# YuxiaWu/RAG4DyG

Measured on AMD Instinct MI355X. Metric: query-seqs/sec encode+top-k over full pool, higher is better.
Workload: dtype f32 (f16x2 operands: two fp16 terms, three products, f32 accumulate)

## Files before the change

rag4dyg_amd/csrc/common.h:

```cpp
#pragma once
#include <hip/hip_runtime.h>
#include <stdint.h>
#include <stdio.h>
#include <stdarg.h>
#include "../../include/r4d.h"
#include "conv1d_route.h"

namespace r4d {

void set_error(const char* fmt, ...);
int dbgflag_kc(); int dbgflag_att(); int dbgflag_sk(); int dbgflag_jac(); int dbgflag_scan(); int dbgflag_s3(); int dbgflag_h2();

#define R4D_REQUIRE(cond, ...)                     \
    do {                                           \
        if (!(cond)) {                             \
            r4d::set_error(__VA_ARGS__);           \
            return R4D_ERR_INVALID;                \
        }                                          \
    } while (0)

#define R4D_HIP(call)                                                                  \
    do {                                                                               \
        hipError_t e_ = (call);                                                        \
        if (e_ != hipSuccess) {                                                        \
// ... 100 lines not shown
bool gemm_skinny_fuses_ln(int M, int K, int N);
void* gemm_skinny_counters(float* scratch, size_t* bytes);
int launch_gemm_skinny(const float* x, const float* wT, const float* bias, const float* resid, int M, int K, int N,
                       int epilogue, float* y, float* scratch, hipStream_t s, const float* ln_w = nullptr,
                       const float* ln_b = nullptr, float ln_eps = 0.f, bool counters_zeroed = false, const float* ln_fold = nullptr);
int launch_fold_layernorm(const float* wT, const float* g, const float* beta, int N, int K, float* wTg, float* lnc, hipStream_t s);

struct S3Args {
    const float* A; const unsigned short* planes; float* C;
    const float* bias; const float* resid;
    int M, N, K, lda, ldc, ldr, epilogue;
    unsigned* kblk; int kb_hd;
};
static inline S3Args s3_args(const float* x, const unsigned short* planes, const float* bias, const float* resid, int M, int K, int N,
                             int epilogue, float* y) {
    S3Args a{};
    a.A = x; a.planes = planes; a.C = y; a.bias = bias; a.resid = resid;
    a.M = M; a.N = N; a.K = K; a.lda = K; a.ldc = N; a.ldr = N; a.epilogue = epilogue;
    return a;
}
int launch_gemm_s3(const S3Args& a, hipStream_t stream);
bool gemm_s3_f32b_supported(int M, int K, int N);
int launch_gemm_s3_f32b(const float* A, const float* B, float* C, int M, int N, int K, int lda, int ldc, int epilogue, hipStream_t stream);
int launch_gemm_s3_scan_order(const float* q_hat, const float* pool_hat, float* scores, int Q, int N, int d, int ng, hipStream_t stream);
int launch_gemm_h2(const S3Args& a, hipStream_t stream);
int launch_split2_planes(const float* w, int N, int K, long long ld_k, long long ld_n, unsigned short* planes, hipStream_t s);
extern int g_gemm_h2p;
bool gemm_h2p_supported(int M, int K, int N);
int launch_gemm_h2p(const S3Args& a, const unsigned short* a_lines, bool out_lines, hipStream_t stream);
int launch_split2_lines(const float* x, long long rows, int K, unsigned short* lines, hipStream_t s);
int launch_gemm_b1(const S3Args& a, hipStream_t stream);
int launch_gemm_b1tn(const float* X, const float* dY, float* out, float* db_out, int I, int J, int M, int lda, int ldb, int S,
                     hipStream_t stream);
int launch_gemm_b1h(const GemmArgs& g, hipStream_t stream);
int launch_gemm_s3tn(const float* X, const float* dY, float* out, float* db_partials, int I, int J, int M, int lda, int ldb, int S,
                     hipStream_t stream);
static inline int gemm_tn_slices(int I, int J, int M, int max_slices) {
    const int tiles = (I / 128) * (J / 256);
    int S = cdiv(512, tiles);
    const int smax = cdiv(M, 256);
    if (S > smax) S = smax;
    if (S > max_slices) S = max_slices;
    return S < 1 ? 1 : S;
}
static inline int tn_row_slices(int M, int S) { return cdiv(M, cdiv(cdiv(M, S), 32) * 32); }
int launch_splitk_reduce(const float* part, long long n4, int S, float* C, hipStream_t stream);
extern int g_encode_bf16;
// ... 39 lines not shown
struct LMLayout { size_t train, h, logits, dh, dwte, tn, ce, total; };
LMLayout lm_layout(const r4d_gpt2_config* cfg, int B, int T, int ldV);
int head_train_step(const char* who, const r4d_gpt2_config* cfg, const r4d_gpt2_weights* w, const r4d_gpt2_grads* grads,
                    const r4d_lm_head* head, int head_mode, float* head_grad, const int64_t* ids_d, const SpliceIn* sp, int B, int T,
                    float gscale, float* loss, float* d_fused, float* hidden_out, const r4d_train_dropout* dropout, void* workspace_d,
                    size_t workspace_bytes, hipStream_t s);

template <typename T> size_t topk_ws_bytes(int rows, int n, int k);
template <typename T>
int topk_rows(const T* vals, const long long* idx_in, int rows, int n, long long ld, int k, long long index_offset, T* out_v,
              long long* out_i, void* ws, size_t ws_bytes, bool counters_zeroed, hipStream_t s);

int launch_layernorm(const float* x, const float* w, const float* b, int rows, int d, float eps, float* y,
                     hipStream_t s);
bool layernorm_lines_supported(int d);
int launch_layernorm_lines(const float* x, const float* w, const float* b, int rows, int d, float eps, unsigned short* y_lines, hipStream_t s);
constexpr int ATT_MAXG = 16;
struct RowGroups {
    int n;
    int B[ATT_MAXG], T[ATT_MAXG];
    const int64_t* ids[ATT_MAXG];
    const float* emb[ATT_MAXG];
};
int launch_embed_layernorm_groups(const RowGroups& G, const float* wte, const float* wpe, int vocab, int d,
                                  const float* w, const float* b, float eps, float* x_out, float* y_out, hipStream_t s, bool y_lines = false);
int launch_causal_softmax(float* S, int nbh, int T, int ld, int row_tile, hipStream_t s);
int launch_embed_pos_layernorm(const int64_t* ids, const float* emb, const int32_t* pos, const float* wte,
                               const float* wpe, int vocab, int n_positions, int t_cap, int B, int d, const float* w,
                               const float* b, float eps, float* x_out, float* y_out, hipStream_t s,
                               void* zero_words = nullptr, size_t zero_bytes = 0);
int launch_decode_attention(const float* qkv_new, float* kv_layer, const int32_t* pos, int B, int t_cap, int H, int d,
                            float* out, hipStream_t s);
struct GreedyState {
    int64_t* next; int32_t* lens; int32_t* pos; int32_t* active; int32_t* gen_len; int32_t* out_tokens;
    const int32_t* params;
    int out_cap, t_cap;
};
struct GreedyEmbed { const float* wte; const float* wpe; float* x_out; unsigned* zero_words; int vocab, n_positions, d, n_zero; };
int launch_greedy_advance(const float* logits, int B, int V, const GreedyState& st, hipStream_t s, const GreedyEmbed* embed = nullptr);
struct AttnGroups {
    int n;
    int seq_prefix[ATT_MAXG + 1];
    int T[ATT_MAXG];
    long long row0[ATT_MAXG];
};
bool attention_h2_supported(int H, int d);
int launch_attention_h2_groups(const unsigned* qkv_words, int n, const int* Bs, const int* Ts, const long long* row0s, int H, int d,
                               float* out, hipStream_t s, bool out_lines = false, const unsigned* kblk = nullptr);
// ... 7 lines not shown
extern int g_attention_variant;
extern int g_attention_fused;
constexpr int PAD_ROWS_HDR = 8;
struct PadRowsPlan {
    int M, Mp, Tmax, Tcap, nblk, ntab, lmax, vocab;
    size_t words() const { return (size_t)PAD_ROWS_HDR + 2 * (size_t)Tcap + lmax + nblk + 2 * (size_t)Mp + vocab; }
    size_t rows() const { return (size_t)Mp + Tcap; }
};
static inline PadRowsPlan pad_rows_plan(size_t M, int Tmax, int vocab) {
    PadRowsPlan p;
    p.M = (int)M; p.Mp = (int)((M + 31) / 32 * 32); p.Tmax = Tmax; p.Tcap = (Tmax + 31) / 32 * 32;
    p.nblk = p.Mp / 32; p.ntab = p.Tcap / 32; p.lmax = (p.nblk + p.ntab + 3) / 4 * 4; p.vocab = vocab;
    return p;
}
struct PadRowsBuf {
    int* hdr; long long* tab_ids; int *list, *drop, *tok, *pos, *hist;
};
static inline PadRowsBuf pad_rows_buf(int* hdr, const PadRowsPlan& p) {
    PadRowsBuf b;
    b.hdr = hdr; b.tab_ids = reinterpret_cast<long long*>(hdr + PAD_ROWS_HDR);
    b.tok = hdr + PAD_ROWS_HDR + 2 * p.Tcap; b.pos = b.tok + p.Mp; b.list = b.pos + p.Mp; b.drop = b.list + p.lmax; b.hist = b.drop + p.nblk;
    return b;
}
int launch_pad_rows_gather(const RowGroups& G, int vocab, long long row_base, const PadRowsBuf& b, hipStream_t s);
int launch_pad_rows_classify(const PadRowsPlan& p, const PadRowsBuf& b, hipStream_t s);
int launch_pad_rows_fill(const PadRowsPlan& p, const PadRowsBuf& b, unsigned* qkv_words, unsigned* kblk, int d, hipStream_t s);
int launch_gemm_h2p_rowmap(const S3Args& a, const unsigned short* a_lines, const PadRowsPlan& p, const PadRowsBuf& b, hipStream_t stream);
constexpr int LNF_ROWS_PER_CHUNK = 16;
size_t lnf_meanpool_scratch_floats(int B, int T, int d);
int launch_lnf_meanpool_groups(const RowGroups& G, const float* x, const float* w, const float* b, int d, float eps,
                               float* hidden_out, float* pool_out, float* scratch, hipStream_t s);

}
```

rag4dyg_amd/csrc/encoder.hip:

```cpp
#include <math.h>
#include <stdlib.h>
#include <string.h>
#include <vector>
#include "common.h"

namespace r4d {

static thread_local char g_err[512] = "";
void set_error(const char* fmt, ...) {
    va_list ap;
    va_start(ap, fmt);
    vsnprintf(g_err, sizeof(g_err), fmt, ap);
    va_end(ap);
}

int g_gemm_split3 = 1;
int g_encode_bf16 = 0;

int conv1d(const Conv1DW& W, const float* x, const float* resid, int M, int epilogue, float* y, hipStream_t s, const Conv1DOpts& opts) {
    const int K = W.in, N = W.out;
    const GemmRoute route = conv1d_route(W, M, epilogue, opts.skinny_scratch != nullptr, opts.bf16);
    switch (route) {
        case ROUTE_B1:
            if (opts.bf16 == BF16_TRAIN) R4D_BRANCH(TB_FWD);
// ... 250 lines not shown
        const r4d_gpt2_layer& L = w->layers[l];
        R4D_REQUIRE(L.ln_1_w && L.c_attn_w && L.attn_proj_w && L.ln_2_w && L.c_fc_w && L.mlp_proj_w,
                    "gpt2: null weight in layer %d", l);
        const Conv1DW Wqkv = conv1d_w(L, C_ATTN, d), Wo = conv1d_w(L, ATTN_PROJ, d), Wfc = conv1d_w(L, C_FC, d), Wp = conv1d_w(L, MLP_PROJ, d);
        const Conv1DOpts enc{nullptr, false, g_encode_bf16 ? BF16_ENCODE : BF16_OFF};
        const bool lines = !g_encode_bf16 && g_gemm_split3 == 2 && g_gemm_h2p && Wqkv.h2 && Wfc.h2 && Wp.h2 && layernorm_lines_supported(d) &&
                           gemm_h2p_supported(M, d, 3 * d) && gemm_h2p_supported(M, d, 4 * d) && gemm_h2p_supported(M, 4 * d, d);
        unsigned short* ln_lines = reinterpret_cast<unsigned short*>(ws.ln);
        unsigned short* fc_lines = reinterpret_cast<unsigned short*>(ws.fc);
        float* qkv = out_qkv_d ? out_qkv_d + (size_t)l * M * 3 * d : ws.qkv;
        bool words = !g_encode_bf16 && !out_qkv_d && g_attention_h2 && g_attention_fused != 0 && g_gemm_split3 == 2 && Wqkv.h2 &&
                     attention_h2_supported(H, d) && gemm_h2_supported(M, d, 3 * d);
        int Bs[ATT_MAXG], Ts[ATT_MAXG], nseq;
        long long r0[ATT_MAXG];
        for (int g0 = 0; g0 < n_groups && words; g0 += ATT_MAXG) {
            attn_chunk(groups, g0, n_groups, Bs, Ts, r0, &nseq);
            if (nseq > 65535) words = false;
        }
        if (g_attention_kblk < 0) { const char* e = getenv("R4D_ATT_KBLK"); g_attention_kblk = e ? atoi(e) != 0 : 1; }
        const bool kblk = words && lines && g_attention_kblk && (d / H) % 32 == 0;
        const bool pad0 = l == 0 && kblk && all_ids && layer0_pad_rows_on() && (3 * d) % 256 == 0 && gemm_h2p_supported((int)pr.rows(), d, 3 * d) &&
                          pr.rows() <= 0x7fffffff / (size_t)(16 * d);
        const PadRowsBuf pb = pad_rows_buf(ws.pad_rows, pr);
        if (pad0) {
            if (hipMemsetAsync(pb.hist, 0, (size_t)pr.vocab * sizeof(int), s) != hipSuccess) { set_error("gpt2: memset of the token counts failed"); return R4D_ERR_HIP; }
            for (int g0 = 0; g0 < n_groups; g0 += ATT_MAXG)
                if ((rc = launch_pad_rows_gather(row_groups(groups, g0, n_groups), cfg->vocab, (long long)groups[g0].row0, pb, s))) return rc;
            if ((rc = launch_pad_rows_classify(pr, pb, s))) return rc;
        }
        if (l == 0) {
            for (int g0 = 0; g0 < n_groups; g0 += ATT_MAXG) {
                const RowGroups R = row_groups(groups, g0, n_groups);
                const size_t r0 = groups[g0].row0;
                rc = launch_embed_layernorm_groups(R, w->wte, w->wpe, cfg->vocab, d, L.ln_1_w, L.ln_1_b, cfg->ln_eps,
                                                   ws.x + r0 * d, ws.ln + r0 * d, s, lines);
                if (rc) return rc;
            }
            if (pad0) {
                RowGroups R = {};
                R.n = 1; R.B[0] = 1; R.T[0] = pr.Tmax; R.ids[0] = reinterpret_cast<const int64_t*>(pb.tab_ids);
                if ((rc = launch_embed_layernorm_groups(R, w->wte, w->wpe, cfg->vocab, d, L.ln_1_w, L.ln_1_b, cfg->ln_eps,
                                                        ws.x + (size_t)pr.Mp * d, ws.ln + (size_t)pr.Mp * d, s, lines))) return rc;
            }
        } else if ((rc = lines ? launch_layernorm_lines(ws.x, L.ln_1_w, L.ln_1_b, M, d, cfg->ln_eps, ln_lines, s)
                               : launch_layernorm(ws.x, L.ln_1_w, L.ln_1_b, M, d, cfg->ln_eps, ws.ln, s))) {
            return rc;
        }
        if (out_layers_d &&
            hipMemcpyAsync(out_layers_d + (size_t)l * M * d, ws.x, (size_t)M * d * sizeof(float),
                           hipMemcpyDeviceToDevice, s) != hipSuccess) {
            set_error("gpt2: layer copy failed");
            return R4D_ERR_HIP;
        }
// ... 338 lines not shown
```

rag4dyg_amd/csrc/encoder_ops.hip:

```cpp
#include <string.h>
#include "common.h"
#include "h2.h"

namespace r4d {

constexpr int MAXV = 32;

__device__ __forceinline__ float wave_sum(float v) {
#pragma unroll
    for (int o = 32; o > 0; o >>= 1) v += __shfl_xor(v, o, 64);
    return v;
}
__device__ __forceinline__ float wave_max(float v) {
#pragma unroll
    for (int o = 32; o > 0; o >>= 1) v = fmaxf(v, __shfl_xor(v, o, 64));
    return v;
}

__device__ __forceinline__ void ln_row(float (&v)[MAXV], int nv, int d, float eps) {
    float s = 0.f;
#pragma unroll
    for (int i = 0; i < MAXV; ++i) if (i < nv) s += v[i];
    const float mean = wave_sum(s) / (float)d;
    float q = 0.f;
// ... 133 lines not shown
    const float* src;
    bool bad = false;
    if (in.ids[g]) {
        const long long id = in.ids[g][local];
        bad = id < 0 || id >= vocab;
        src = wte + (bad ? 0 : id) * (long long)d;
    } else {
        src = in.emb[g] + local * d;
    }
    const float* pe = wpe + (local % G.T[g]) * d;
#pragma unroll
    for (int i = 0; i < MAXV; ++i)
        if (i < nv) {
            const float e = src[lane + 64 * i] + pe[lane + 64 * i];
            v[i] = bad ? __builtin_nanf("") : e;
            x_out[row * d + lane + 64 * i] = v[i];
        }
    ln_row(v, nv, d, eps);
#pragma unroll
    for (int i = 0; i < MAXV; ++i)
        if (i < nv) y_out[row * d + lane + 64 * i] = v[i] * w[lane + 64 * i] + b[lane + 64 * i];
}

template <int NQ, bool LINES = false>
__global__ __launch_bounds__(256) void embed_ln4_groups_kernel(const RowTable G, const RowInputs in,
                                                               const float* __restrict__ wte, const float* __restrict__ wpe,
                                                               int vocab, int d, const float* __restrict__ w,
                                                               const float* __restrict__ b, float eps,
                                                               float* __restrict__ x_out, float* __restrict__ y_out) {
    const int lane = threadIdx.x & 63;
    const long long row = (long long)blockIdx.x * 4 + (threadIdx.x >> 6);
    if (row >= G.row_prefix[G.n]) return;
    int g = 0;
    while (g + 1 < G.n && row >= G.row_prefix[g + 1]) ++g;
    const long long local = row - G.row_prefix[g];
    const int nq = d >> 8;
    const float* src;
    bool bad = false;
    if (in.ids[g]) {
        const long long id = in.ids[g][local];
        bad = id < 0 || id >= vocab;
        src = wte + (bad ? 0 : id) * (long long)d;
    } else {
        src = in.emb[g] + local * d;
    }
    const float4* s4 = reinterpret_cast<const float4*>(src) + lane;
    const float4* p4 = reinterpret_cast<const float4*>(wpe + (local % G.T[g]) * d) + lane;
    float4* xr = reinterpret_cast<float4*>(x_out + row * d) + lane;
    float4 v[NQ];
#pragma unroll
    for (int i = 0; i < NQ; ++i) {
        v[i] = make_float4(0.f, 0.f, 0.f, 0.f);
        if (i < nq) {
            const float4 e = s4[64 * i], q = p4[64 * i];
            const float nan = __builtin_nanf("");
            v[i] = bad ? make_float4(nan, nan, nan, nan) : make_float4(e.x + q.x, e.y + q.y, e.z + q.z, e.w + q.w);
            xr[64 * i] = v[i];
        }
    }
    float s_ = 0.f;
#pragma unroll
    for (int i = 0; i < NQ; ++i) s_ += (v[i].x + v[i].y) + (v[i].z + v[i].w);
    const float mean = wave_sum(s_) / (float)d;
    float q = 0.f;
#pragma unroll
    for (int i = 0; i < NQ; ++i)
        if (i < nq) {
            const float a0 = v[i].x - mean, a1 = v[i].y - mean, a2 = v[i].z - mean, a3 = v[i].w - mean;
            q += (a0 * a0 + a1 * a1) + (a2 * a2 + a3 * a3);
        }
    const float rstd = rsqrtf(wave_sum(q) / (float)d + eps);
    float4* yr = reinterpret_cast<float4*>(y_out + row * d) + lane;
#pragma unroll
    for (int i = 0; i < NQ; ++i)
        if (i < nq) {
            const float4 ww = reinterpret_cast<const float4*>(w)[lane + 64 * i], bb = reinterpret_cast<const float4*>(b)[lane + 64 * i];
            const float4 y4 = make_float4((v[i].x - mean) * rstd * ww.x + bb.x, (v[i].y - mean) * rstd * ww.y + bb.y,
                                          (v[i].z - mean) * rstd * ww.z + bb.z, (v[i].w - mean) * rstd * ww.w + bb.w);
            if constexpr (LINES) store_lines4(y_out, row, d, 4 * lane + 256 * i, y4.x, y4.y, y4.z, y4.w);
            else yr[64 * i] = y4;
        }
}

int launch_embed_layernorm_groups(const RowGroups& G, const float* wte, const float* wpe, int vocab, int d,
                                  const float* w, const float* b, float eps, float* x_out, float* y_out, hipStream_t s, bool y_lines) {
    R4D_REQUIRE(d % 64 == 0 && d <= 64 * MAXV, "embed: d=%d must be a multiple of 64 and <= %d", d, 64 * MAXV);
    R4D_REQUIRE(G.n >= 1 && G.n <= ATT_MAXG, "embed: %d batches per launch (max %d)", G.n, ATT_MAXG);
    const RowTable t = make_table(G);
    const long long rows = t.row_prefix[G.n];
    if (rows <= 0) return R4D_OK;
    RowInputs in;
    for (int g = 0; g < ATT_MAXG; ++g) { in.ids[g] = g < G.n ? G.ids[g] : nullptr; in.emb[g] = g < G.n ? G.emb[g] : nullptr; }
    ProfScope prof(PK_EMBED_LN, 12.0 * rows * d + 8.0 * rows, s);
    uintptr_t align = (uintptr_t)wte | (uintptr_t)wpe | (uintptr_t)w | (uintptr_t)b | (uintptr_t)x_out | (uintptr_t)y_out;
    for (int g = 0; g < G.n; ++g) align |= (uintptr_t)in.emb[g];
    const bool vec = d % 256 == 0 && (align & 15) == 0;
    const dim3 grid((unsigned)cdiv(rows, 4));
    if (y_lines) {
        R4D_REQUIRE(vec, "embed: line output needs d %% 256 == 0 and 16-byte aligned pointers");
        R4D_BRANCH(EMBED_LN4);
        if (d <= 512) hipLaunchKernelGGL((embed_ln4_groups_kernel<2, true>), grid, dim3(256), 0, s, t, in, wte, wpe, vocab, d, w, b, eps, x_out, y_out);
        else if (d <= 1024) hipLaunchKernelGGL((embed_ln4_groups_kernel<4, true>), grid, dim3(256), 0, s, t, in, wte, wpe, vocab, d, w, b, eps, x_out, y_out);
        else hipLaunchKernelGGL((embed_ln4_groups_kernel<8, true>), grid, dim3(256), 0, s, t, in, wte, wpe, vocab, d, w, b, eps, x_out, y_out);
        R4D_CHECK_LAUNCH("embed_layernorm");
        return R4D_OK;
    }
    if (vec && d <= 512) { R4D_BRANCH(EMBED_LN4); hipLaunchKernelGGL(embed_ln4_groups_kernel<2>, grid, dim3(256), 0, s, t, in, wte, wpe, vocab, d, w, b, eps, x_out, y_out); }
    else if (vec && d <= 1024) { R4D_BRANCH(EMBED_LN4); hipLaunchKernelGGL(embed_ln4_groups_kernel<4>, grid, dim3(256), 0, s, t, in, wte, wpe, vocab, d, w, b, eps, x_out, y_out); }
    else if (vec) { R4D_BRANCH(EMBED_LN4); hipLaunchKernelGGL(embed_ln4_groups_kernel<8>, grid, dim3(256), 0, s, t, in, wte, wpe, vocab, d, w, b, eps, x_out, y_out); }
    else {
        R4D_BRANCH(EMBED_GENERIC);
        hipLaunchKernelGGL(embed_ln_groups_kernel, grid, dim3(256), 0, s, t, in, wte, wpe, vocab, d, w, b, eps, x_out, y_out);
    }
    R4D_CHECK_LAUNCH("embed_layernorm");
    return R4D_OK;
}

__global__ __launch_bounds__(256) void embed_pos_ln_kernel(const int64_t* __restrict__ ids, const float* __restrict__ emb,
                                                           const int32_t* __restrict__ pos, const float* __restrict__ wte,
                                                           const float* __restrict__ wpe, int vocab, int n_positions,
                                                           int t_cap, int B, int d, const float* __restrict__ w,
                                                           const float* __restrict__ b, float eps,
                                                           float* __restrict__ x_out, float* __restrict__ y_out,
                                                           unsigned* __restrict__ zero_words, int n_zero) {
    if (blockIdx.x == 0)
        for (int i = threadIdx.x; i < n_zero; i += 256) zero_words[i] = 0u;
    const int lane = threadIdx.x & 63;
    const int row = blockIdx.x * 4 + (threadIdx.x >> 6);
    if (row >= B) return;
    const int nv = d >> 6;
    const int p = pos[row];
    bool bad = p < 0 || p >= n_positions || p >= t_cap;
// ... 354 lines not shown
        else hipLaunchKernelGGL(lnf_partial_kernel<32>, grid, dim3(256), 4 * d * sizeof(float), s, t, x, w, b, d, eps, hidden_out, part, g_range_flag);
        R4D_CHECK_LAUNCH("lnf_partial");
    }
    if (pool_out) {
        ProfScope prof(PK_MEANPOOL_REDUCE, 4.0 * parts * d + 4.0 * nseq * d, s);
        hipLaunchKernelGGL(meanpool_reduce_kernel, dim3(nseq), dim3(256), 0, s, t, scratch, d, pool_out);
        R4D_CHECK_LAUNCH("meanpool_reduce");
    }
    return R4D_OK;
}

__global__ __launch_bounds__(256) void pad_rows_gather_kernel(const RowTable G, const RowInputs in, int vocab, long long row_base,
                                                              int* __restrict__ tok, int* __restrict__ pos, int* __restrict__ hist) {
    const long long row = (long long)blockIdx.x * 256 + threadIdx.x;
    if (row >= G.row_prefix[G.n]) return;
    int g = 0;
    while (g + 1 < G.n && row >= G.row_prefix[g + 1]) ++g;
    const long long local = row - G.row_prefix[g];
    const long long id = in.ids[g][local];
    const bool ok = id >= 0 && id < vocab;
    const int t = (int)(local % G.T[g]);
    tok[row_base + row] = ok ? (int)id : -1;
    pos[row_base + row] = t;
    if (ok && t == G.T[g] - 1) atomicAdd(&hist[id], 1);
}

__global__ __launch_bounds__(1024) void pad_rows_classify_kernel(const PadRowsPlan p, const PadRowsBuf b) {
    __shared__ unsigned long long red[1024];
    __shared__ int scan[1024];
    __shared__ int base[2];
    const int tid = threadIdx.x;
    unsigned long long best = 0;
    for (int v = tid; v < p.vocab; v += 1024) {
        const unsigned long long key = ((unsigned long long)(unsigned)b.hist[v] << 32) | (0xffffffffu - (unsigned)v);
        best = key > best ? key : best;
    }
    red[tid] = best;
    if (tid == 0) { base[0] = 0; base[1] = 0; }
    __syncthreads();
    for (int o = 512; o > 0; o >>= 1) {
        if (tid < o) red[tid] = red[tid + o] > red[tid] ? red[tid + o] : red[tid];
        __syncthreads();
    }
    const int c = (int)(0xffffffffu - (unsigned)(red[0] & 0xffffffffu));
    for (int t = tid; t < p.Tcap; t += 1024) b.tab_ids[t] = c;
    for (int b0 = 0; b0 < p.nblk; b0 += 1024) {
        const int blk = b0 + tid;
        bool kept = false, in = blk < p.nblk;
        if (in) {
            kept = blk * 32 + 32 > p.M;
            if (!kept) {
                const int4* t4 = reinterpret_cast<const int4*>(b.tok + blk * 32);
#pragma unroll
                for (int i = 0; i < 8; ++i) { const int4 v = t4[i]; kept |= (v.x != c) | (v.y != c) | (v.z != c) | (v.w != c); }
            }
        }
        scan[tid] = kept ? 1 : 0;
// ... 23 lines not shown
    }
}

__global__ __launch_bounds__(256) void pad_rows_fill_kernel(const PadRowsPlan p, const PadRowsBuf b, uint4* __restrict__ qkv,
                                                            uint4* __restrict__ kblk, int d) {
    if ((int)blockIdx.x >= b.hdr[1]) return;
    const int blk = b.drop[blockIdx.x];
    __shared__ int prow[32];
    if (threadIdx.x < 32) prow[threadIdx.x] = p.Mp + min(b.pos[blk * 32 + threadIdx.x], p.Tcap - 1);
    __syncthreads();
    const int dq = d / 4;
    for (int i = threadIdx.x; i < 32 * dq; i += 256) {
        const int r = i / dq, j = i - r * dq;
        const long long dst = (long long)(blk * 32 + r) * (3 * dq) + j, src = (long long)prow[r] * (3 * dq) + j;
        qkv[dst] = qkv[src];
        qkv[dst + 2 * dq] = qkv[src + 2 * dq];
    }
    for (int i = threadIdx.x; i < 32 * dq; i += 256) {
        const int ch = i >> 5, r = i & 31, sr = prow[r];
        kblk[((long long)blk * dq + ch) * 32 + r] = kblk[((long long)(sr >> 5) * dq + ch) * 32 + (sr & 31)];
    }
}

int launch_pad_rows_gather(const RowGroups& G, int vocab, long long row_base, const PadRowsBuf& b, hipStream_t s) {
    R4D_REQUIRE(G.n >= 1 && G.n <= ATT_MAXG, "pad_rows: %d batches per launch (max %d)", G.n, ATT_MAXG);
    const RowTable t = make_table(G);
    const long long rows = t.row_prefix[G.n];
    if (rows <= 0) return R4D_OK;
    RowInputs in;
    for (int g = 0; g < ATT_MAXG; ++g) { in.ids[g] = g < G.n ? G.ids[g] : nullptr; in.emb[g] = nullptr; }
    for (int g = 0; g < G.n; ++g) R4D_REQUIRE(in.ids[g], "pad_rows: batches given as embeddings have no tokens to classify");
    ProfScope prof(PK_PAD_CLASSIFY, 16.0 * rows, s);
    hipLaunchKernelGGL(pad_rows_gather_kernel, dim3((unsigned)cdiv(rows, 256)), dim3(256), 0, s, t, in, vocab, row_base, b.tok, b.pos, b.hist);
    R4D_CHECK_LAUNCH("pad_rows_gather");
    return R4D_OK;
}

int launch_pad_rows_classify(const PadRowsPlan& p, const PadRowsBuf& b, hipStream_t s) {
    ProfScope prof(PK_PAD_CLASSIFY, 4.0 * p.Mp + 4.0 * p.vocab + 8.0 * p.nblk, s);
    hipLaunchKernelGGL(pad_rows_classify_kernel, dim3(1), dim3(1024), 0, s, p, b);
    R4D_CHECK_LAUNCH("pad_rows_classify");
    return R4D_OK;
}

int launch_pad_rows_fill(const PadRowsPlan& p, const PadRowsBuf& b, unsigned* qkv_words, unsigned* kblk, int d, hipStream_t s) {
    R4D_REQUIRE(qkv_words && kblk && d % 32 == 0 && ((((uintptr_t)qkv_words | (uintptr_t)kblk)) & 15) == 0, "pad_rows_fill: bad arguments");
    ProfScope prof(PK_PAD_FILL, 24.0 * p.Mp * d, s);
    hipLaunchKernelGGL(pad_rows_fill_kernel, dim3(p.nblk), dim3(256), 0, s, p, b, reinterpret_cast<uint4*>(qkv_words),
                       reinterpret_cast<uint4*>(kblk), d);
    R4D_CHECK_LAUNCH("pad_rows_fill");
    return R4D_OK;
}

}
```

rag4dyg_amd/csrc/gemm_s3.hip:

```cpp
#include <stdlib.h>
#include <string.h>
#include <atomic>
#include "bf16x3.h"

#ifndef S3_NRS
#define S3_NRS 1
#endif
#ifndef S3_DBG
#define S3_DBG 0
#endif

namespace r4d {

struct S3Shape {
    int M, N, K, lda, ldc, ldr;
    int plane_bytes;
};

__global__ __launch_bounds__(256) void split3_planes_kernel(const float* __restrict__ w, int N, int K, long long ld_k,
                                                            long long ld_n, unsigned short* __restrict__ planes) {
    __shared__ float tile[32][33];
    const int n0 = blockIdx.x * 32, k0 = blockIdx.y * 32;
    const int tx = threadIdx.x & 31, ty = threadIdx.x >> 5;
    const bool n_fast = ld_n == 1;
// ... 18 lines not shown

template <int BM, int BN, int WGM, int WGN, int NBUF, int NRS, int EPI, bool BF32 = false, int SCAN = 0>
__global__ __launch_bounds__(64 * WGM * WGN, (WGM * WGN) / 4) void gemm_s3_kernel(
    const float* __restrict__ Ag, const unsigned short* __restrict__ Bp, float* __restrict__ Cg,
    const float* __restrict__ biasg, const float* __restrict__ residg, const S3Shape g) {
    constexpr int BK = 32;
    constexpr int NTHREADS = 64 * WGM * WGN;
    constexpr int WM = BM / WGM, WN = BN / WGN, TM = WM / 32, TN = WN / 32;
    constexpr int NIA = BM * 4 / NTHREADS, NIB = BN * 4 / NTHREADS;
    constexpr int A_PLANE = BM * 4, B_PLANE = BN * 4;
    constexpr int STAGE = 3 * (A_PLANE + B_PLANE);
    constexpr int D = NBUF - 1;
    static_assert(NIA >= 1 && NIB >= 1 && NIA <= 2 && NIB <= 2 && TM >= 1 && TN >= 1 && (NBUF == 2 || NBUF == 3), "tile");
    static_assert(NRS == 1 || (NRS == 2 && NBUF == 2), "two register stages: with the two-stage LDS ring only");
    __shared__ u32x4 lds[NBUF * STAGE];

    int m0, n0;
    grouped_tile<BM, BN>(g.M, g.N, m0, n0);
    const int nkt = g.K / BK;

    const int tid = threadIdx.x, lane = tid & 63, wid = tid >> 6;
    const int wm = wid / WGN, wn = wid % WGN;
    const int li = lane & 31, lh = lane >> 5;

    int a_off[NIA], b_off[NIB], a_dst[NIA], b_dst[NIB];
#pragma unroll
    for (int i = 0; i < NIA; ++i) {
        const int idx = tid + i * NTHREADS, row = idx >> 2, c = idx & 3;
        a_off[i] = (min(m0 + row, g.M - 1) * g.lda + (SCAN ? (c >> 1) * 16 + (c & 1) * 4 : c * 8)) * 4;
        a_dst[i] = row * 4 + (c ^ ((row >> 2) & 3));
    }
#pragma unroll
    for (int i = 0; i < NIB; ++i) {
        const int idx = tid + i * NTHREADS, row = idx >> 2, c = idx & 3;
        b_off[i] = (min(n0 + row, g.N - 1) * g.K + (SCAN ? (c >> 1) * 16 + (c & 1) * 4 : c * 8)) * (BF32 ? 4 : 2);
        b_dst[i] = row * 4 + (c ^ ((row >> 2) & 3));
    }
    const __amdgpu_buffer_rsrc_t a_rsrc = __builtin_amdgcn_make_buffer_rsrc(
        const_cast<float*>(Ag), 0, (int)(((long long)(g.M - 1) * g.lda + g.K) * 4), 0x00020000);
    const __amdgpu_buffer_rsrc_t b_rsrc = __builtin_amdgcn_make_buffer_rsrc(
        const_cast<unsigned short*>(Bp), 0, BF32 ? (int)((long long)g.N * g.K * 4) : 3 * g.plane_bytes, 0x00020000);

    u32x4 ra[NRS][NIA][2], rb[NRS][NIB][3];
    static_assert(SCAN == 0 || BF32, "scan order: with the fp32 second operand only");
    constexpr int P2 = SCAN ? 32 : 16;
    const int scan_kw = SCAN ? nkt / (SCAN ? SCAN : 1) : 1;
// ... 420 lines not shown
}

bool gemm_s3_f32b_supported(int M, int K, int N) {
    return gemm_s3_supported(M, K, N) && (long long)N * K * 4 < (1ll << 31);
}
int launch_gemm_s3_f32b(const float* A, const float* B, float* C, int M, int N, int K, int lda, int ldc, int epilogue, hipStream_t stream) {
    R4D_REQUIRE(A && B && C && gemm_s3_f32b_supported(M, K, N), "gemm_s3_f32b: unsupported shape M=%d K=%d N=%d", M, K, N);
    R4D_REQUIRE(lda % 4 == 0 && ((uintptr_t)A % 16) == 0 && ((uintptr_t)B % 16) == 0, "gemm_s3_f32b: alignment");
    R4D_BRANCH(S3_F32B);
    const int tiles = cdiv(M, 128) * cdiv(N, 256);
    ProfScope prof(PK_GEMM_S3_128x256, 2.0 * (double)M * N * K, stream);
    S3Shape sh;
    sh.M = M; sh.N = N; sh.K = K; sh.lda = lda; sh.ldc = ldc; sh.ldr = ldc; sh.plane_bytes = 0;
    const unsigned short* Bp = reinterpret_cast<const unsigned short*>(B);
    if (epilogue == EPI_HALF_PLUS)
        hipLaunchKernelGGL((gemm_s3_kernel<128, 256, 2, 4, 2, 1, EPI_HALF_PLUS, true>), dim3(tiles), dim3(512), 0, stream, A, Bp, C, nullptr, nullptr, sh);
    else if (epilogue == EPI_NONE)
        hipLaunchKernelGGL((gemm_s3_kernel<128, 256, 2, 4, 2, 1, EPI_NONE, true>), dim3(tiles), dim3(512), 0, stream, A, Bp, C, nullptr, nullptr, sh);
    else { set_error("gemm_s3_f32b: epilogue %d has no instantiation", epilogue); return R4D_ERR_INVALID; }
    R4D_CHECK_LAUNCH("gemm_s3_f32b");
    return R4D_OK;
}

int launch_gemm_s3_scan_order(const float* q_hat, const float* pool_hat, float* scores, int Q, int N, int d, int ng, hipStream_t stream) {
    if (!gemm_s3_f32b_supported(Q, d, N) || ng < 2 || ng > 4 || (d / 32) % ng != 0) return 1;
    if ((((uintptr_t)q_hat | (uintptr_t)pool_hat) & 15u) != 0 || d % 4 != 0) return 1;
    R4D_BRANCH(SCAN_TILED);
    const int tiles = cdiv(Q, 128) * cdiv(N, 256);
    S3Shape sh;
    sh.M = Q; sh.N = N; sh.K = d; sh.lda = d; sh.ldc = N; sh.ldr = N; sh.plane_bytes = 0;
    const unsigned short* Bp = reinterpret_cast<const unsigned short*>(pool_hat);
#define S3_SCAN_LAUNCH_(NG_) hipLaunchKernelGGL((gemm_s3_kernel<128, 256, 2, 4, 2, 1, EPI_HALF_PLUS, true, NG_>), dim3(tiles), dim3(512), 0, stream, q_hat, Bp, scores, nullptr, nullptr, sh)
    switch (ng) {
        case 2: S3_SCAN_LAUNCH_(2); break;
        case 3: S3_SCAN_LAUNCH_(3); break;
        default: S3_SCAN_LAUNCH_(4); break;
    }
#undef S3_SCAN_LAUNCH_
    R4D_CHECK_LAUNCH("gemm_s3_scan_order");
    return R4D_OK;
}

int launch_split3_planes(const float* w, int N, int K, long long ld_k, long long ld_n, unsigned short* planes, hipStream_t s) {
    R4D_REQUIRE(w && planes && N >= 1 && K >= 1, "split3_planes: bad arguments");
    R4D_REQUIRE(ld_n == 1 || ld_k == 1, "split3_planes: one of the two strides must be 1");
    hipLaunchKernelGGL(split3_planes_kernel, dim3(cdiv(N, 32), cdiv(K, 32)), dim3(256), 0, s, w, N, K, ld_k, ld_n, planes);
    R4D_CHECK_LAUNCH("split3_planes");
    return R4D_OK;
}

int dbgflag_s3() { return S3_DBG != 0; }

}

using namespace r4d;
// ... 15 lines not shown
```

rag4dyg_amd/csrc/score.hip:

```cpp
#include <math.h>
#include <string.h>
#include <stdlib.h>
#include "bf16x3.h"

#ifndef SCAN_RING_P
#define SCAN_RING_P 3
#endif
#ifndef SCAN_DBG
#define SCAN_DBG 0
#endif

namespace r4d {

int dbgflag_scan() { return SCAN_DBG != 0; }

__global__ __launch_bounds__(256) void normalize_rows_kernel(const float* __restrict__ x, int n, int d,
                                                             float* __restrict__ out, unsigned* __restrict__ range_flag) {
    const int lane = threadIdx.x & 63;
    const int row = blockIdx.x * 4 + (threadIdx.x >> 6);
    if (row >= n) return;
    const float* p = x + (long long)row * d;
    float s = 0.f;
    for (int c = lane; c < d; c += 64) s += p[c] * p[c];
#pragma unroll
// ... 683 lines not shown
    }
    R4D_CHECK_LAUNCH("pool_scan");
    return R4D_OK;
}

template <int KW, int NG>
static int launch_scan_variant(const float* qhat, const float* pool, int Q, int N, float* scores, unsigned* zero_d, int nzero,
                               hipStream_t s) {
    if (g_gemm_split3) { R4D_BRANCH(SCAN_BF16X3); return launch_scan_variant_p<KW, NG, true>(qhat, pool, Q, N, scores, zero_d, nzero, s); }
    R4D_BRANCH(SCAN_F32);
    return launch_scan_variant_p<KW, NG, false>(qhat, pool, Q, N, scores, zero_d, nzero, s);
}

static int launch_pool_scan(const float* qhat, const float* pool, int Q, int N, int d, float* scores, unsigned* zero_d,
                            int nzero, hipStream_t s) {
    static int kw8 = -1;
    if (kw8 < 0) { const char* e = getenv("R4D_SCAN_KW8"); kw8 = e ? atoi(e) : 1; }
    if (d != 32 && d != 64 && d != 128 && d != 256 && d != 384 && d != 512 && d != 768 && d != 1024) return 1;
    ProfScope prof(PK_POOL_SCAN, 4.0 * N * d * cdiv(Q, 32) + 4.0 * Q * d + 4.0 * (double)Q * N, s);
    static int tiled = -1;
    if (tiled < 0) { const char* e = getenv("R4D_SCAN_TILED"); tiled = e ? atoi(e) : 1; }
    if (tiled && Q >= 64 && g_gemm_split3 && (long long)cdiv(Q, 128) * cdiv(N, 256) >= 192) {
        const int ng = d == 256 ? 2 : d == 384 ? 3 : d == 512 ? (kw8 ? 2 : 4) : d == 768 ? 3 : d == 1024 ? 4 : 1;
        if (nzero > 0) R4D_HIP(hipMemsetAsync(zero_d, 0, (size_t)nzero * sizeof(unsigned), s));
        const int rc = launch_gemm_s3_scan_order(qhat, pool, scores, Q, N, d, ng, s);
        if (rc <= 0) return rc;
    }
    switch (d) {
        case 32:   R4D_BRANCH(SCAN_1_1); return launch_scan_variant<1, 1>(qhat, pool, Q, N, scores, zero_d, nzero, s);
        case 64:   R4D_BRANCH(SCAN_2_1); return launch_scan_variant<2, 1>(qhat, pool, Q, N, scores, zero_d, nzero, s);
        case 128:  R4D_BRANCH(SCAN_4_1); return launch_scan_variant<4, 1>(qhat, pool, Q, N, scores, zero_d, nzero, s);
        case 256:  R4D_BRANCH(SCAN_4_2); return launch_scan_variant<4, 2>(qhat, pool, Q, N, scores, zero_d, nzero, s);
        case 384:  R4D_BRANCH(SCAN_4_3); return launch_scan_variant<4, 3>(qhat, pool, Q, N, scores, zero_d, nzero, s);
        case 512:  if (kw8) { R4D_BRANCH(SCAN_8_2); return launch_scan_variant<8, 2>(qhat, pool, Q, N, scores, zero_d, nzero, s); }
                   R4D_BRANCH(SCAN_4_4); return launch_scan_variant<4, 4>(qhat, pool, Q, N, scores, zero_d, nzero, s);
        case 768:  R4D_BRANCH(SCAN_8_3); return launch_scan_variant<8, 3>(qhat, pool, Q, N, scores, zero_d, nzero, s);
        case 1024: R4D_BRANCH(SCAN_8_4); return launch_scan_variant<8, 4>(qhat, pool, Q, N, scores, zero_d, nzero, s);
        default:   return 1;
    }
}

}

using namespace r4d;

extern "C" {

int r4d_normalize_rows_f32(const float* x_d, int32_t n, int32_t d, float* out_d, void* stream) {
// ... 55 lines not shown
```

Measured before the change: 40470.

## Fold pad-row counts, table embed and scan zeroing into existing kernels

```diff
diff --git a/rag4dyg_amd/csrc/common.h b/rag4dyg_amd/csrc/common.h
--- a/rag4dyg_amd/csrc/common.h
+++ b/rag4dyg_amd/csrc/common.h
@@ -146,7 +146,8 @@
 int launch_gemm_s3(const S3Args& a, hipStream_t stream);
 bool gemm_s3_f32b_supported(int M, int K, int N);
 int launch_gemm_s3_f32b(const float* A, const float* B, float* C, int M, int N, int K, int lda, int ldc, int epilogue, hipStream_t stream);
-int launch_gemm_s3_scan_order(const float* q_hat, const float* pool_hat, float* scores, int Q, int N, int d, int ng, hipStream_t stream);
+int launch_gemm_s3_scan_order(const float* q_hat, const float* pool_hat, float* scores, int Q, int N, int d, int ng, unsigned* zero_d, int nzero,
+                              hipStream_t stream);
 int launch_gemm_h2(const S3Args& a, hipStream_t stream);
 int launch_split2_planes(const float* w, int N, int K, long long ld_k, long long ld_n, unsigned short* planes, hipStream_t s);
 extern int g_gemm_h2p;
@@ -232,8 +233,11 @@
     const int64_t* ids[ATT_MAXG];
     const float* emb[ATT_MAXG];
 };
+struct PadRowsPlan;
+struct PadRowsBuf;
 int launch_embed_layernorm_groups(const RowGroups& G, const float* wte, const float* wpe, int vocab, int d,
-                                  const float* w, const float* b, float eps, float* x_out, float* y_out, hipStream_t s, bool y_lines = false);
+                                  const float* w, const float* b, float eps, float* x_out, float* y_out, hipStream_t s, bool y_lines = false,
+                                  const PadRowsPlan* plan = nullptr, const PadRowsBuf* pbuf = nullptr);
 int launch_causal_softmax(float* S, int nbh, int T, int ld, int row_tile, hipStream_t s);
 int launch_embed_pos_layernorm(const int64_t* ids, const float* emb, const int32_t* pos, const float* wte,
                                const float* wpe, int vocab, int n_positions, int t_cap, int B, int d, const float* w,
@@ -287,8 +291,10 @@
     b.tok = hdr + PAD_ROWS_HDR + 2 * p.Tcap; b.pos = b.tok + p.Mp; b.list = b.pos + p.Mp; b.drop = b.list + p.lmax; b.hist = b.drop + p.nblk;
     return b;
 }
-int launch_pad_rows_gather(const RowGroups& G, int vocab, long long row_base, const PadRowsBuf& b, hipStream_t s);
-int launch_pad_rows_classify(const PadRowsPlan& p, const PadRowsBuf& b, hipStream_t s);
+int launch_pad_rows_gather(const RowGroups& G, int vocab, long long row_base, const PadRowsBuf& b, bool count, hipStream_t s);
+constexpr int PAD_ROWS_LDS_VOCAB = 12288;
+bool pad_rows_lds_hist(int n_groups, int vocab);
+int launch_pad_rows_classify(const PadRowsPlan& p, const PadRowsBuf& b, const RowGroups* all, hipStream_t s);
 int launch_pad_rows_fill(const PadRowsPlan& p, const PadRowsBuf& b, unsigned* qkv_words, unsigned* kblk, int d, hipStream_t s);
 int launch_gemm_h2p_rowmap(const S3Args& a, const unsigned short* a_lines, const PadRowsPlan& p, const PadRowsBuf& b, hipStream_t stream);
 constexpr int LNF_ROWS_PER_CHUNK = 16;
diff --git a/rag4dyg_amd/csrc/encoder.hip b/rag4dyg_amd/csrc/encoder.hip
--- a/rag4dyg_amd/csrc/encoder.hip
+++ b/rag4dyg_amd/csrc/encoder.hip
@@ -296,13 +296,21 @@
         const bool pad0 = l == 0 && kblk && all_ids && layer0_pad_rows_on() && (3 * d) % 256 == 0 && gemm_h2p_supported((int)pr.rows(), d, 3 * d) &&
                           pr.rows() <= 0x7fffffff / (size_t)(16 * d);
         const PadRowsBuf pb = pad_rows_buf(ws.pad_rows, pr);
+        const bool lds_hist = pad0 && pad_rows_lds_hist(n_groups, pr.vocab), one_embed = pad0 && n_groups < ATT_MAXG;
         if (pad0) {
-            if (hipMemsetAsync(pb.hist, 0, (size_t)pr.vocab * sizeof(int), s) != hipSuccess) { set_error("gpt2: memset of the token counts failed"); return R4D_ERR_HIP; }
+            if (!lds_hist && hipMemsetAsync(pb.hist, 0, (size_t)pr.vocab * sizeof(int), s) != hipSuccess) { set_error("gpt2: memset of the token counts failed"); return R4D_ERR_HIP; }
             for (int g0 = 0; g0 < n_groups; g0 += ATT_MAXG)
-                if ((rc = launch_pad_rows_gather(row_groups(groups, g0, n_groups), cfg->vocab, (long long)groups[g0].row0, pb, s))) return rc;
-            if ((rc = launch_pad_rows_classify(pr, pb, s))) return rc;
-        }
-        if (l == 0) {
+                if ((rc = launch_pad_rows_gather(row_groups(groups, g0, n_groups), cfg->vocab, (long long)groups[g0].row0, pb, !lds_hist, s))) return rc;
+            const RowGroups all = row_groups(groups, 0, n_groups);
+            if ((rc = launch_pad_rows_classify(pr, pb, lds_hist ? &all : nullptr, s))) return rc;
+        }
+        if (l == 0 && one_embed) {
+            RowGroups R = row_groups(groups, 0, n_groups);
+            R.B[R.n] = 1; R.T[R.n] = pr.Tmax; R.ids[R.n] = reinterpret_cast<const int64_t*>(pb.tab_ids); R.emb[R.n] = nullptr;
+            ++R.n;
+            if ((rc = launch_embed_layernorm_groups(R, w->wte, w->wpe, cfg->vocab, d, L.ln_1_w, L.ln_1_b, cfg->ln_eps, ws.x, ws.ln, s, lines,
+                                                    &pr, &pb))) return rc;
+        } else if (l == 0) {
             for (int g0 = 0; g0 < n_groups; g0 += ATT_MAXG) {
                 const RowGroups R = row_groups(groups, g0, n_groups);
                 const size_t r0 = groups[g0].row0;
diff --git a/rag4dyg_amd/csrc/encoder_ops.hip b/rag4dyg_amd/csrc/encoder_ops.hip
--- a/rag4dyg_amd/csrc/encoder_ops.hip
+++ b/rag4dyg_amd/csrc/encoder_ops.hip
@@ -179,18 +179,24 @@
         if (i < nv) y_out[row * d + lane + 64 * i] = v[i] * w[lane + 64 * i] + b[lane + 64 * i];
 }
 
-template <int NQ, bool LINES = false>
+struct EmbedPadRows { const int* hdr; const int* tok; int M; long long tab_shift; };
+template <int NQ, bool LINES = false, bool PLAN = false>
 __global__ __launch_bounds__(256) void embed_ln4_groups_kernel(const RowTable G, const RowInputs in,
                                                                const float* __restrict__ wte, const float* __restrict__ wpe,
                                                                int vocab, int d, const float* __restrict__ w,
                                                                const float* __restrict__ b, float eps,
-                                                               float* __restrict__ x_out, float* __restrict__ y_out) {
+                                                               float* __restrict__ x_out, float* __restrict__ y_out, const EmbedPadRows pr) {
     const int lane = threadIdx.x & 63;
-    const long long row = (long long)blockIdx.x * 4 + (threadIdx.x >> 6);
+    long long row = (long long)blockIdx.x * 4 + (threadIdx.x >> 6);
     if (row >= G.row_prefix[G.n]) return;
     int g = 0;
     while (g + 1 < G.n && row >= G.row_prefix[g + 1]) ++g;
     const long long local = row - G.row_prefix[g];
+    bool no_line = false;
+    if constexpr (PLAN) {
+        if (g == G.n - 1) row += pr.tab_shift;
+        else if ((row | 31) < pr.M) no_line = __all(pr.tok[(row & ~31ll) + (lane & 31)] == pr.hdr[2]);
+    }
     const int nq = d >> 8;
     const float* src;
     bool bad = false;
@@ -215,6 +221,7 @@
             xr[64 * i] = v[i];
         }
     }
+    if (PLAN && no_line) return;
     float s_ = 0.f;
 #pragma unroll
     for (int i = 0; i < NQ; ++i) s_ += (v[i].x + v[i].y) + (v[i].z + v[i].w);
@@ -240,7 +247,8 @@
 }
 
 int launch_embed_layernorm_groups(const RowGroups& G, const float* wte, const float* wpe, int vocab, int d,
-                                  const float* w, const float* b, float eps, float* x_out, float* y_out, hipStream_t s, bool y_lines) {
+                                  const float* w, const float* b, float eps, float* x_out, float* y_out, hipStream_t s, bool y_lines,
+                                  const PadRowsPlan* plan, const PadRowsBuf* pbuf) {
     R4D_REQUIRE(d % 64 == 0 && d <= 64 * MAXV, "embed: d=%d must be a multiple of 64 and <= %d", d, 64 * MAXV);
     R4D_REQUIRE(G.n >= 1 && G.n <= ATT_MAXG, "embed: %d batches per launch (max %d)", G.n, ATT_MAXG);
     const RowTable t = make_table(G);
@@ -253,18 +261,30 @@
     for (int g = 0; g < G.n; ++g) align |= (uintptr_t)in.emb[g];
     const bool vec = d % 256 == 0 && (align & 15) == 0;
     const dim3 grid((unsigned)cdiv(rows, 4));
+    const EmbedPadRows none = {nullptr, nullptr, 0, 0};
+    if (plan) {
+        R4D_REQUIRE(y_lines && vec && pbuf && G.n >= 2 && G.B[G.n - 1] == 1 && rows - G.T[G.n - 1] == plan->M && G.T[G.n - 1] <= plan->Tcap,
+                    "embed: the pad-row plan needs line output, the call's %d rows and the table as the last batch", plan->M);
+        const EmbedPadRows pr = {pbuf->hdr, pbuf->tok, plan->M, (long long)plan->Mp - plan->M};
+        R4D_BRANCH(EMBED_LN4);
+        if (d <= 512) hipLaunchKernelGGL((embed_ln4_groups_kernel<2, true, true>), grid, dim3(256), 0, s, t, in, wte, wpe, vocab, d, w, b, eps, x_out, y_out, pr);
+        else if (d <= 1024) hipLaunchKernelGGL((embed_ln4_groups_kernel<4, true, true>), grid, dim3(256), 0, s, t, in, wte, wpe, vocab, d, w, b, eps, x_out, y_out, pr);
+        else hipLaunchKernelGGL((embed_ln4_groups_kernel<8, true, true>), grid, dim3(256), 0, s, t, in, wte, wpe, vocab, d, w, b, eps, x_out, y_out, pr);
+        R4D_CHECK_LAUNCH("embed_layernorm");
+        return R4D_OK;
+    }
     if (y_lines) {
         R4D_REQUIRE(vec, "embed: line output needs d %% 256 == 0 and 16-byte aligned pointers");
         R4D_BRANCH(EMBED_LN4);
-        if (d <= 512) hipLaunchKernelGGL((embed_ln4_groups_kernel<2, true>), grid, dim3(256), 0, s, t, in, wte, wpe, vocab, d, w, b, eps, x_out, y_out);
-        else if (d <= 1024) hipLaunchKernelGGL((embed_ln4_groups_kernel<4, true>), grid, dim3(256), 0, s, t, in, wte, wpe, vocab, d, w, b, eps, x_out, y_out);
-        else hipLaunchKernelGGL((embed_ln4_groups_kernel<8, true>), grid, dim3(256), 0, s, t, in, wte, wpe, vocab, d, w, b, eps, x_out, y_out);
+        if (d <= 512) hipLaunchKernelGGL((embed_ln4_groups_kernel<2, true>), grid, dim3(256), 0, s, t, in, wte, wpe, vocab, d, w, b, eps, x_out, y_out, none);
+        else if (d <= 1024) hipLaunchKernelGGL((embed_ln4_groups_kernel<4, true>), grid, dim3(256), 0, s, t, in, wte, wpe, vocab, d, w, b, eps, x_out, y_out, none);
+        else hipLaunchKernelGGL((embed_ln4_groups_kernel<8, true>), grid, dim3(256), 0, s, t, in, wte, wpe, vocab, d, w, b, eps, x_out, y_out, none);
         R4D_CHECK_LAUNCH("embed_layernorm");
         return R4D_OK;
     }
-    if (vec && d <= 512) { R4D_BRANCH(EMBED_LN4); hipLaunchKernelGGL(embed_ln4_groups_kernel<2>, grid, dim3(256), 0, s, t, in, wte, wpe, vocab, d, w, b, eps, x_out, y_out); }
-    else if (vec && d <= 1024) { R4D_BRANCH(EMBED_LN4); hipLaunchKernelGGL(embed_ln4_groups_kernel<4>, grid, dim3(256), 0, s, t, in, wte, wpe, vocab, d, w, b, eps, x_out, y_out); }
-    else if (vec) { R4D_BRANCH(EMBED_LN4); hipLaunchKernelGGL(embed_ln4_groups_kernel<8>, grid, dim3(256), 0, s, t, in, wte, wpe, vocab, d, w, b, eps, x_out, y_out); }
+    if (vec && d <= 512) { R4D_BRANCH(EMBED_LN4); hipLaunchKernelGGL(embed_ln4_groups_kernel<2>, grid, dim3(256), 0, s, t, in, wte, wpe, vocab, d, w, b, eps, x_out, y_out, none); }
+    else if (vec && d <= 1024) { R4D_BRANCH(EMBED_LN4); hipLaunchKernelGGL(embed_ln4_groups_kernel<4>, grid, dim3(256), 0, s, t, in, wte, wpe, vocab, d, w, b, eps, x_out, y_out, none); }
+    else if (vec) { R4D_BRANCH(EMBED_LN4); hipLaunchKernelGGL(embed_ln4_groups_kernel<8>, grid, dim3(256), 0, s, t, in, wte, wpe, vocab, d, w, b, eps, x_out, y_out, none); }
     else {
         R4D_BRANCH(EMBED_GENERIC);
         hipLaunchKernelGGL(embed_ln_groups_kernel, grid, dim3(256), 0, s, t, in, wte, wpe, vocab, d, w, b, eps, x_out, y_out);
@@ -665,17 +685,30 @@
     const int t = (int)(local % G.T[g]);
     tok[row_base + row] = ok ? (int)id : -1;
     pos[row_base + row] = t;
-    if (ok && t == G.T[g] - 1) atomicAdd(&hist[id], 1);
-}
-
-__global__ __launch_bounds__(1024) void pad_rows_classify_kernel(const PadRowsPlan p, const PadRowsBuf b) {
+    if (hist && ok && t == G.T[g] - 1) atomicAdd(&hist[id], 1);
+}
+
+template <bool LDS_HIST>
+__global__ __launch_bounds__(1024) void pad_rows_classify_kernel(const PadRowsPlan p, const PadRowsBuf b, const RowTable G) {
     __shared__ unsigned long long red[1024];
+    __shared__ int lhist[LDS_HIST ? PAD_ROWS_LDS_VOCAB : 1];
     __shared__ int scan[1024];
     __shared__ int base[2];
     const int tid = threadIdx.x;
+    if constexpr (LDS_HIST) {
+        for (int v = tid; v < p.vocab; v += 1024) lhist[v] = 0;
+        __syncthreads();
+        for (int seq = tid; seq < G.seq_prefix[G.n]; seq += 1024) {
+            int g = 0;
+            while (g + 1 < G.n && seq >= G.seq_prefix[g + 1]) ++g;
+            const int id = b.tok[G.row0_of(g, seq - G.seq_prefix[g]) + G.T[g] - 1];
+            if (id >= 0) atomicAdd(&lhist[id], 1);
+        }
+        __syncthreads();
+    }
     unsigned long long best = 0;
     for (int v = tid; v < p.vocab; v += 1024) {
-        const unsigned long long key = ((unsigned long long)(unsigned)b.hist[v] << 32) | (0xffffffffu - (unsigned)v);
+        const unsigned long long key = ((unsigned long long)(unsigned)(LDS_HIST ? lhist[v] : b.hist[v]) << 32) | (0xffffffffu - (unsigned)v);
         best = key > best ? key : best;
     }
     red[tid] = best;
@@ -745,7 +778,9 @@
     }
 }
 
-int launch_pad_rows_gather(const RowGroups& G, int vocab, long long row_base, const PadRowsBuf& b, hipStream_t s) {
+bool pad_rows_lds_hist(int n_groups, int vocab) { return n_groups <= ATT_MAXG && vocab <= PAD_ROWS_LDS_VOCAB; }
+
+int launch_pad_rows_gather(const RowGroups& G, int vocab, long long row_base, const PadRowsBuf& b, bool count, hipStream_t s) {
     R4D_REQUIRE(G.n >= 1 && G.n <= ATT_MAXG, "pad_rows: %d batches per launch (max %d)", G.n, ATT_MAXG);
     const RowTable t = make_table(G);
     const long long rows = t.row_prefix[G.n];
@@ -754,14 +789,21 @@
     for (int g = 0; g < ATT_MAXG; ++g) { in.ids[g] = g < G.n ? G.ids[g] : nullptr; in.emb[g] = nullptr; }
     for (int g = 0; g < G.n; ++g) R4D_REQUIRE(in.ids[g], "pad_rows: batches given as embeddings have no tokens to classify");
     ProfScope prof(PK_PAD_CLASSIFY, 16.0 * rows, s);
-    hipLaunchKernelGGL(pad_rows_gather_kernel, dim3((unsigned)cdiv(rows, 256)), dim3(256), 0, s, t, in, vocab, row_base, b.tok, b.pos, b.hist);
+    hipLaunchKernelGGL(pad_rows_gather_kernel, dim3((unsigned)cdiv(rows, 256)), dim3(256), 0, s, t, in, vocab, row_base, b.tok, b.pos,
+                       count ? b.hist : nullptr);
     R4D_CHECK_LAUNCH("pad_rows_gather");
     return R4D_OK;
 }
 
-int launch_pad_rows_classify(const PadRowsPlan& p, const PadRowsBuf& b, hipStream_t s) {
+int launch_pad_rows_classify(const PadRowsPlan& p, const PadRowsBuf& b, const RowGroups* all, hipStream_t s) {
     ProfScope prof(PK_PAD_CLASSIFY, 4.0 * p.Mp + 4.0 * p.vocab + 8.0 * p.nblk, s);
-    hipLaunchKernelGGL(pad_rows_classify_kernel, dim3(1), dim3(1024), 0, s, p, b);
+    if (all) {
+        R4D_REQUIRE(pad_rows_lds_hist(all->n, p.vocab), "pad_rows_classify: %d batches / vocab %d do not fit the LDS counts", all->n, p.vocab);
+        hipLaunchKernelGGL(pad_rows_classify_kernel<true>, dim3(1), dim3(1024), 0, s, p, b, make_table(*all));
+    } else {
+        RowGroups none = {};
+        hipLaunchKernelGGL(pad_rows_classify_kernel<false>, dim3(1), dim3(1024), 0, s, p, b, make_table(none));
+    }
     R4D_CHECK_LAUNCH("pad_rows_classify");
     return R4D_OK;
 }
diff --git a/rag4dyg_amd/csrc/gemm_s3.hip b/rag4dyg_amd/csrc/gemm_s3.hip
--- a/rag4dyg_amd/csrc/gemm_s3.hip
+++ b/rag4dyg_amd/csrc/gemm_s3.hip
@@ -64,6 +64,12 @@
     const int tid = threadIdx.x, lane = tid & 63, wid = tid >> 6;
     const int wm = wid / WGN, wn = wid % WGN;
     const int li = lane & 31, lh = lane >> 5;
+
+    if constexpr (SCAN != 0) {
+        unsigned* zero_d = reinterpret_cast<unsigned*>(const_cast<float*>(residg));
+        if (blockIdx.x == 0 && zero_d)
+            for (int i = tid; i < g.ldr; i += NTHREADS) zero_d[i] = 0u;
+    }
 
     int a_off[NIA], b_off[NIB], a_dst[NIA], b_dst[NIB];
 #pragma unroll
@@ -530,15 +536,16 @@
     return R4D_OK;
 }
 
-int launch_gemm_s3_scan_order(const float* q_hat, const float* pool_hat, float* scores, int Q, int N, int d, int ng, hipStream_t stream) {
+int launch_gemm_s3_scan_order(const float* q_hat, const float* pool_hat, float* scores, int Q, int N, int d, int ng, unsigned* zero_d, int nzero,
+                              hipStream_t stream) {
     if (!gemm_s3_f32b_supported(Q, d, N) || ng < 2 || ng > 4 || (d / 32) % ng != 0) return 1;
     if ((((uintptr_t)q_hat | (uintptr_t)pool_hat) & 15u) != 0 || d % 4 != 0) return 1;
     R4D_BRANCH(SCAN_TILED);
     const int tiles = cdiv(Q, 128) * cdiv(N, 256);
     S3Shape sh;
-    sh.M = Q; sh.N = N; sh.K = d; sh.lda = d; sh.ldc = N; sh.ldr = N; sh.plane_bytes = 0;
+    sh.M = Q; sh.N = N; sh.K = d; sh.lda = d; sh.ldc = N; sh.ldr = zero_d ? nzero : 0; sh.plane_bytes = 0;
     const unsigned short* Bp = reinterpret_cast<const unsigned short*>(pool_hat);
-#define S3_SCAN_LAUNCH_(NG_) hipLaunchKernelGGL((gemm_s3_kernel<128, 256, 2, 4, 2, 1, EPI_HALF_PLUS, true, NG_>), dim3(tiles), dim3(512), 0, stream, q_hat, Bp, scores, nullptr, nullptr, sh)
+#define S3_SCAN_LAUNCH_(NG_) hipLaunchKernelGGL((gemm_s3_kernel<128, 256, 2, 4, 2, 1, EPI_HALF_PLUS, true, NG_>), dim3(tiles), dim3(512), 0, stream, q_hat, Bp, scores, nullptr, reinterpret_cast<const float*>(zero_d), sh)
     switch (ng) {
         case 2: S3_SCAN_LAUNCH_(2); break;
         case 3: S3_SCAN_LAUNCH_(3); break;
diff --git a/rag4dyg_amd/csrc/score.hip b/rag4dyg_amd/csrc/score.hip
--- a/rag4dyg_amd/csrc/score.hip
+++ b/rag4dyg_amd/csrc/score.hip
@@ -729,8 +729,7 @@
     if (tiled < 0) { const char* e = getenv("R4D_SCAN_TILED"); tiled = e ? atoi(e) : 1; }
     if (tiled && Q >= 64 && g_gemm_split3 && (long long)cdiv(Q, 128) * cdiv(N, 256) >= 192) {
         const int ng = d == 256 ? 2 : d == 384 ? 3 : d == 512 ? (kw8 ? 2 : 4) : d == 768 ? 3 : d == 1024 ? 4 : 1;
-        if (nzero > 0) R4D_HIP(hipMemsetAsync(zero_d, 0, (size_t)nzero * sizeof(unsigned), s));
-        const int rc = launch_gemm_s3_scan_order(qhat, pool, scores, Q, N, d, ng, s);
+        const int rc = launch_gemm_s3_scan_order(qhat, pool, scores, Q, N, d, ng, zero_d, nzero, s);
         if (rc <= 0) return rc;
     }
     switch (d) {
```

Result: no change. 40610, median of 6 (+0.4%).
